# BUTSpeechFIT/VBx

Measured on NVIDIA H100. Metric: x-vectors/sec through 10 VB-HMM EM iters, higher is better.
Workload: dtype f32

## Files before the change

vbx_b200/csrc/vbx_capi.cu:

```cuda
#include <dlfcn.h>
#include <nvtx3/nvToolsExt.h>

#include <algorithm>
#include <cmath>
#include <cstdio>
#include <cstring>
#include <numeric>
#include <string>
#include <vector>

#include "../../include/vbx_b200.h"
#include "vbx_internal.cuh"

struct vbx_handle_s {
    int device = 0;
    int sms = 0;
    std::string err;
    vbx::Plan plan;
    vbx::Workspace ws;
    bool planned = false, bound = false, prepared = false;
    bool f64_only = false;
    size_t ws_need = 0;
    void *plan_mem = nullptr;
    int opt_fb_spl = 0;
    int opt_fb_classic = 0;
    int opt_projection = 0;
    int opt_timing = 0;
    int opt_gemm = 0;
    int opt_debug_sync = 0;
    int opt_fb_split = 0;
    int opt_exact_stop = 1;
    int64_t launches = 0;
    cudaStream_t hi_stream = nullptr;
    cudaEvent_t ev_fork = nullptr, ev_join = nullptr;
    int opt_graph = 0;
    cudaStream_t graph_stream = nullptr;
    cudaEvent_t ev_g0 = nullptr, ev_g1 = nullptr;
    cudaGraphExec_t graph_exec = nullptr;
    uint64_t graph_key = 0, seen_key = 0;
    int64_t graph_launches = 0;
    bool graph_broken = false;
    void *nccl_comm = nullptr;
    int nccl_ranks = 1;
    int (*nccl_allreduce)(const void *, void *, size_t, int, int, void *, cudaStream_t) = nullptr;
    std::vector<int64_t> offsets_host;
    std::vector<int64_t> ahc_d_off;
    size_t ahc_need = 0;
    std::vector<cudaEvent_t> ev_pool;
    size_t ev_used = 0;
    std::vector<int> ev_class;
    double t_ms[VBX_N_KERNEL_CLASSES] = {0};
    int64_t t_cnt[VBX_N_KERNEL_CLASSES] = {0};
};

namespace {

int fail(vbx_handle_t h, int code, const std::string &msg) {
    if (h) h->err = msg;
    return code;
}
int cuda_fail(vbx_handle_t h, cudaError_t e, const char *what) {
    return fail(h, VBX_ERR_CUDA, std::string(what) + ": " + cudaGetErrorString(e));
}
size_t align_up(size_t v, size_t a = 256) { return (v + a - 1) / a * a; }

struct Range {
    explicit Range(const char *name) { nvtxRangePushA(name); }
    ~Range() { nvtxRangePop(); }
};

struct DeviceGuard {
    int prev = -1;
    cudaError_t err = cudaSuccess;
    explicit DeviceGuard(int device) {
        if (cudaGetDevice(&prev) != cudaSuccess) prev = -1;
        if (prev != device) err = cudaSetDevice(device);
    }
    ~DeviceGuard() {
// ... 115 lines not shown
    h->device = device;
    h->sms = prop.multiProcessorCount;
    {
        DeviceGuard guard(device);
        int lo = 0, hi = 0;
        if (guard.err != cudaSuccess || cudaDeviceGetStreamPriorityRange(&lo, &hi) != cudaSuccess ||
            cudaStreamCreateWithPriority(&h->hi_stream, cudaStreamNonBlocking, hi) != cudaSuccess ||
            cudaEventCreateWithFlags(&h->ev_fork, cudaEventDisableTiming) != cudaSuccess ||
            cudaEventCreateWithFlags(&h->ev_join, cudaEventDisableTiming) != cudaSuccess ||
            cudaStreamCreateWithFlags(&h->graph_stream, cudaStreamNonBlocking) != cudaSuccess ||
            cudaEventCreateWithFlags(&h->ev_g0, cudaEventDisableTiming) != cudaSuccess ||
            cudaEventCreateWithFlags(&h->ev_g1, cudaEventDisableTiming) != cudaSuccess) {
            vbx_destroy(h);
            return VBX_ERR_CUDA;
        }
    }
    *out = h;
    return VBX_OK;
}

int vbx_destroy(vbx_handle_t h) {
    if (!h) return VBX_ERR_ARG;
    DeviceGuard guard(h->device);
    if (h->plan_mem) cudaFree(h->plan_mem);
    if (h->hi_stream) cudaStreamDestroy(h->hi_stream);
    if (h->ev_fork) cudaEventDestroy(h->ev_fork);
    if (h->ev_join) cudaEventDestroy(h->ev_join);
    if (h->graph_exec) cudaGraphExecDestroy(h->graph_exec);
    if (h->graph_stream) cudaStreamDestroy(h->graph_stream);
    if (h->ev_g0) cudaEventDestroy(h->ev_g0);
    if (h->ev_g1) cudaEventDestroy(h->ev_g1);
    for (cudaEvent_t e : h->ev_pool) cudaEventDestroy(e);
    delete h;
    return VBX_OK;
}

const char *vbx_last_error(vbx_handle_t h) { return h ? h->err.c_str() : "null handle"; }

int vbx_set_option(vbx_handle_t h, const char *name, int32_t value) {
    if (!h || !name) return VBX_ERR_ARG;
    drop_graph(h);
    if (!strcmp(name, "graph")) {
        if (value < 0 || value > 2) return fail(h, VBX_ERR_ARG, "graph must be 0 (auto), 1 (always) or 2 (never)");
        h->opt_graph = value;
        return VBX_OK;
    }
    if (!strcmp(name, "fb_states_per_lane")) {
        if (value != 0 && value != 1 && value != 2 && value != 4) return fail(h, VBX_ERR_ARG, "fb_states_per_lane must be 0,1,2,4");
        h->opt_fb_spl = value;
        return VBX_OK;
    }
    if (!strcmp(name, "fb_classic")) {
        h->opt_fb_classic = value ? 1 : 0;
        return VBX_OK;
    }
    if (!strcmp(name, "gemm")) {
        if (value != 0 && value != 1) return fail(h, VBX_ERR_ARG, "gemm must be 0 (mma 3xTF32) or 1 (FFMA)");
        h->opt_gemm = value;
        return VBX_OK;
    }
    if (!strcmp(name, "debug_sync")) {
        h->opt_debug_sync = value ? 1 : 0;
        return VBX_OK;
    }
    if (!strcmp(name, "fb_split")) {
        if (value < 0 || value > 2) return fail(h, VBX_ERR_ARG, "fb_split must be 0 (auto), 1 (always) or 2 (never)");
        h->opt_fb_split = value;
        return VBX_OK;
    }
    if (!strcmp(name, "exact_stop")) {
        h->opt_exact_stop = value ? 1 : 0;
        return VBX_OK;
    }
    if (!strcmp(name, "timing")) {
        h->opt_timing = value ? 1 : 0;
        return VBX_OK;
    }
    if (!strcmp(name, "projection")) {
        if (value < 0 || value > 2) return fail(h, VBX_ERR_ARG, "projection must be 0,1,2");
        h->opt_projection = value;
        return VBX_OK;
    }
    return fail(h, VBX_ERR_ARG, std::string("unknown option ") + name);
}

int vbx_plan(vbx_handle_t h, const int64_t *offsets_host, int32_t n_rec, int32_t R, int32_t S,
             size_t *workspace_bytes_out) {
    if (!h || !offsets_host || n_rec < 0) return fail(h, VBX_ERR_ARG, "vbx_plan: null argument");
    if (R < 4 || R > vbx::kMaxR || (R & 3)) return fail(h, VBX_ERR_ARG, "vbx_plan: R must be a multiple of 4 in [4,128]");
    if (S != 4 && S != 8 && S != 16 && S != 32 && S != 64 && S != vbx::kMaxSWide)
        return fail(h, VBX_ERR_ARG, "vbx_plan: S must come from vbx_padded_states() or vbx_padded_states_wide()");
    if (S == vbx::kMaxSWide && h->opt_fb_split == 2)
        return fail(h, VBX_ERR_ARG, "vbx_plan: S = 128 plans always take the split forward-backward schedule (there is no fused "
                                    "sweep at 128 states), so option fb_split = 2 (never) cannot be honoured");
    if (n_rec > 0 && offsets_host[0] != 0) return fail(h, VBX_ERR_ARG, "vbx_plan: offsets[0] must be 0");
    for (int b = 0; b < n_rec; ++b) {
        const int64_t T = offsets_host[b + 1] - offsets_host[b];
        if (T < 0) return fail(h, VBX_ERR_ARG, "vbx_plan: offsets must be non-decreasing");
        if (T > (int64_t)1 << 30) return fail(h, VBX_ERR_ARG, "vbx_plan: recording longer than 2^30 frames");
    }
    DeviceGuard guard(h->device);
    cudaError_t e = guard.err;
    if (e != cudaSuccess) return cuda_fail(h, e, "cudaSetDevice");

    std::vector<int32_t> order(n_rec);
    std::iota(order.begin(), order.end(), 0);
// ... 305 lines not shown
    if (warm_start && (!alpha_io || !invL_io)) return fail(h, VBX_ERR_ARG, w + ": warm_start needs alpha_io and invL_io");
    const vbx::Plan &pl = h->plan;
    if (pl.n_rec == 0) return VBX_OK;
    if (!Li_out || !n_iters_out || !flags_out || !pi_io) return fail(h, VBX_ERR_ARG, w + ": null output pointer");
    if (pl.n_frames && (!rho || !Phi || !gamma_io)) return fail(h, VBX_ERR_ARG, w + ": null pointer");
    vbx::RunParams rp;
    rp.epsilon = epsilon;
    rp.max_iters = max_iters;
    rp.hybrid = (pl.exact && epsilon > -1e300 && epsilon < 1e300 && max_iters > 1) ? 1 : 0;
    rp.warm = warm_start ? 1 : 0;

    auto enqueue = [&](cudaStream_t st) -> int {
    int rc = 0;
    {
        Timed t(h, st, VBX_K_RUN_INIT);
        rc = counted(h, vbx::launch_run_init(pl, h->ws, gamma_io, n_states, Li_out, n_iters_out, flags_out, max_iters, Fa, Fb,
                                             loop_prob, Fa_v, Fb_v, loopP_v, st), "run_init");
    }
    if (rc) return rc;
    const int rounds = max_iters + (rp.hybrid ? 1 : 0);
    const bool fb_hi = !pl.split && pl.n_rec >= 1024;
    for (int it = 0; it < rounds; ++it) {
        Range nvtx_iter("vbx_em_iteration");
        const bool given = it == 0 && warm_start;
        if (it < max_iters) {
            if (rp.hybrid) {
                Timed t(h, st, VBX_K_EXACT64);
                rc = counted(h, vbx::launch_snapshot(pl, h->ws, gamma_io, pi_io, it, st), "snapshot");
                if (rc) return rc;
            }
            if (!given) {
                Timed t(h, st, VBX_K_MSTEP);
                rc = counted(h, h->opt_gemm ? vbx::launch_mstep_partial(pl, h->ws, rho, gamma_io, st)
                                            : vbx::launch_mstep_mma(pl, h->ws, rho, gamma_io, st), "mstep_partial");
            }
            if (rc) return rc;
            {
                Timed t(h, st, VBX_K_SPEAKER_MODEL);
                rc = counted(h, vbx::launch_speaker_model(pl, h->ws, Phi, n_states, alpha_io, invL_io, given, st), "speaker_model");
            }
            if (rc) return rc;
            {
                Timed t(h, st, VBX_K_LOGLIK);
                rc = counted(h, h->opt_gemm ? vbx::launch_loglik(pl, h->ws, rho, pi_io, n_states, st) : vbx::launch_loglik_mma(pl, h->ws, rho, pi_io, n_states, st), "loglik");
            }
            if (rc) return rc;
            if (fb_hi) {
                cudaEventRecord(h->ev_fork, st);
                cudaStreamWaitEvent(h->hi_stream, h->ev_fork, 0);
            }
            {
                cudaStream_t fs = fb_hi ? h->hi_stream : st;
                Timed t(h, fs, VBX_K_FWDBWD);
                rc = counted(h, vbx::launch_forward_backward(pl, h->ws, rp, gamma_io, pi_io, n_states, Li_out, n_iters_out, flags_out, it, h->opt_fb_spl, h->opt_fb_classic, fs), "forward_backward");
            }
            if (fb_hi) {
                cudaEventRecord(h->ev_join, h->hi_stream);
                cudaStreamWaitEvent(st, h->ev_join, 0);
            }
            if (rc) return rc;
        }
        if (rp.hybrid && it > 0) {
            Timed t(h, st, VBX_K_EXACT64);
            rc = counted(h, vbx::launch_exact64_round(pl, h->ws, rp, rho, Phi, gamma_io, pi_io, n_states, alpha_io, invL_io, Li_out,
                                                      n_iters_out, flags_out, st), "exact64");
            if (rc) return rc;
        }
    }
    return VBX_OK;
    };

    cudaStream_t user = (cudaStream_t)stream;
    const bool want_graph = (h->opt_graph == 1 || (h->opt_graph == 0 && pl.split)) && !h->opt_timing && !h->opt_debug_sync &&
                            !h->graph_broken;
    if (!want_graph) return enqueue(user);
    uint64_t key = 1469598103934665603ull;
    auto mix = [&](uint64_t v) { key = (key ^ v) * 1099511628211ull; };
    auto bits = [](double d) { uint64_t u; memcpy(&u, &d, 8); return u; };
    for (const void *p : {(const void *)rho, (const void *)Phi, (const void *)gamma_io, (const void *)pi_io, (const void *)n_states,
                          (const void *)alpha_io, (const void *)invL_io, (const void *)Li_out, (const void *)n_iters_out,
                          (const void *)flags_out, (const void *)h->ws.p, (const void *)Fa_v, (const void *)Fb_v,
                          (const void *)loopP_v})
        mix((uint64_t)(uintptr_t)p);
    mix(bits(Fa)); mix(bits(Fb)); mix(bits(loop_prob)); mix(bits(epsilon)); mix((uint64_t)max_iters); mix((uint64_t)warm_start);
    if (key == 0) key = 1;
    auto replay = [&]() -> int {
        cudaEventRecord(h->ev_g0, user);
        cudaStreamWaitEvent(h->graph_stream, h->ev_g0, 0);
        const cudaError_t e = cudaGraphLaunch(h->graph_exec, h->graph_stream);
        cudaEventRecord(h->ev_g1, h->graph_stream);
        cudaStreamWaitEvent(user, h->ev_g1, 0);
        if (e != cudaSuccess) return cuda_fail(h, e, "cudaGraphLaunch");
        return VBX_OK;
    };
    if (h->graph_exec && key == h->graph_key) {
        h->launches += h->graph_launches;
        return replay();
    }
    if (key != h->seen_key) {
        h->seen_key = key;
        return enqueue(user);
    }
    drop_graph(h);
    h->seen_key = key;
    const int64_t before = h->launches;
    if (cudaStreamBeginCapture(h->graph_stream, cudaStreamCaptureModeRelaxed) != cudaSuccess) {
        cudaGetLastError();
// ... 571 lines not shown
```

vbx_b200/csrc/vbx_internal.cuh:

```cuda
#pragma once
#include <cuda_runtime.h>
#include <stdint.h>

#include <string>
#include <vector>

#define VBX_EPS_TR 1e-8f

namespace vbx {

constexpr int kLTile = 64;
constexpr int kMTile = 512;
constexpr int kLongT = 4096;
constexpr int kChunk = 256;
constexpr int kMaxR = 128;
constexpr int kMaxS = 64;
constexpr int kMaxSWide = 128;
constexpr int kTcMaxD = 2048;

struct Plan {
    int32_t n_rec = 0, R = 0, S = 0;
    int32_t exact = 0;
    int32_t split = 0;
    int64_t n_frames = 0;
// ... 88 lines not shown
    return r;
}
template <>
__device__ __forceinline__ Vec<4> ld_vec<4>(const float *p) {
    float4 t = *reinterpret_cast<const float4 *>(p);
    Vec<4> r;
    r.v[0] = t.x;
    r.v[1] = t.y;
    r.v[2] = t.z;
    r.v[3] = t.w;
    return r;
}
template <int N>
__device__ __forceinline__ Vec<N> ldg_vec(const float *p);
template <>
__device__ __forceinline__ Vec<1> ldg_vec<1>(const float *p) {
    Vec<1> r;
    r.v[0] = __ldg(p);
    return r;
}
template <>
__device__ __forceinline__ Vec<2> ldg_vec<2>(const float *p) {
    float2 t = __ldg(reinterpret_cast<const float2 *>(p));
    Vec<2> r;
    r.v[0] = t.x;
    r.v[1] = t.y;
    return r;
}
template <>
__device__ __forceinline__ Vec<4> ldg_vec<4>(const float *p) {
    float4 t = __ldg(reinterpret_cast<const float4 *>(p));
    Vec<4> r;
    r.v[0] = t.x;
    r.v[1] = t.y;
    r.v[2] = t.z;
    r.v[3] = t.w;
    return r;
}
template <int N>
__device__ __forceinline__ void st_vec(float *p, const float *v);
template <>
__device__ __forceinline__ void st_vec<1>(float *p, const float *v) {
    *p = v[0];
}
template <>
__device__ __forceinline__ void st_vec<2>(float *p, const float *v) {
    *reinterpret_cast<float2 *>(p) = make_float2(v[0], v[1]);
}
template <>
__device__ __forceinline__ void st_vec<4>(float *p, const float *v) {
    *reinterpret_cast<float4 *>(p) = make_float4(v[0], v[1], v[2], v[3]);
}

__device__ __forceinline__ int find_problem(const int64_t *__restrict__ pref, int G, int64_t x) {
    int lo = 0, hi = G;
    while (hi - lo > 1) {
        const int mid = (lo + hi) >> 1;
        if (pref[mid] <= x) lo = mid;
        else hi = mid;
    }
    return lo;
}

#endif

int launch_prepare_scale(const Plan &pl, const Workspace &ws, const float *fea, const float *Phi, float *rho,
                         cudaStream_t st);
int launch_project_ffma(const Plan &pl, const float *X, int D, const float *V, float *rho, cudaStream_t st);
int launch_g_from_rho(const Plan &pl, const Workspace &ws, const float *rho, const float *Phi, cudaStream_t st);
int launch_run_init(const Plan &pl, const Workspace &ws, const float *gamma, const int32_t *n_states, double *Li,
                    int32_t *n_iters, int32_t *flags, int max_iters, double Fa, double Fb, double loopP,
                    const double *Fa_v, const double *Fb_v, const double *loopP_v, cudaStream_t st);
int launch_mstep_partial(const Plan &pl, const Workspace &ws, const float *rho, const float *gamma, cudaStream_t st);
int launch_speaker_model(const Plan &pl, const Workspace &ws, const float *Phi,
                         const int32_t *n_states, float *alpha_io, float *invL_io, bool from_given,
                         cudaStream_t st);
int launch_loglik(const Plan &pl, const Workspace &ws, const float *rho, const float *pi, const int32_t *n_states,
                  cudaStream_t st);
int launch_forward_backward(const Plan &pl, const Workspace &ws, const RunParams &rp, float *gamma, float *pi,
                            const int32_t *n_states, double *Li, int32_t *n_iters, int32_t *flags, int iter,
                            int spl, int classic, cudaStream_t st);
int launch_elbo_trace(const Plan &pl, const double *Li, int max_iters, double *out, cudaStream_t st);
int launch_forward_backward_split(const Plan &pl, const Workspace &ws, const RunParams &rp, float *gamma, float *pi,
                                  const int32_t *n_states, int spl, cudaStream_t st);
int launch_forward_backward_long(const Plan &pl, const Workspace &ws, const RunParams &rp, float *gamma, float *pi,
                                 const int32_t *n_states, cudaStream_t st);
int launch_mstep_mma(const Plan &pl, const Workspace &ws, const float *rho, const float *gamma, cudaStream_t st);
int launch_loglik_mma(const Plan &pl, const Workspace &ws, const float *rho, const float *pi, const int32_t *n_states,
                      cudaStream_t st);
int launch_snapshot(const Plan &pl, const Workspace &ws, const float *gamma, const float *pi, int iter, cudaStream_t st);
int launch_exact64_round(const Plan &pl, const Workspace &ws, const RunParams &rp, const float *rho, const float *Phi,
                         float *gamma, float *pi, const int32_t *n_states, float *alpha_io, float *invL_io, double *Li,
                         int32_t *n_iters, int32_t *flags, cudaStream_t st);
size_t f64_workspace_bytes(const Plan &pl);
int launch_run_f64(const Plan &pl, void *workspace, const double *fea, const double *Phi, double *gamma, double *pi,
                   const int32_t *n_states, double Fa, double Fb, double loopP, int max_iters, double epsilon,
                   double *alpha_io, double *invL_io, int warm, double *Li, int32_t *n_iters, int32_t *flags,
                   cudaStream_t st);
int launch_hard_labels(const Plan &pl, const float *gamma, const int32_t *n_states, int32_t *first, int32_t *second,
                       cudaStream_t st);
int launch_hard_labels_keep(const Plan &pl, const float *gamma, const int32_t *n_states, const int32_t *keep,
                            int32_t *first, int32_t *second, double *mass, cudaStream_t st);
int launch_init_turns(const Plan &pl, const int64_t *seg, const int64_t *spk_off, const int64_t *turn_off,
                      const int64_t *turn_lo, const int64_t *turn_hi, const int64_t *turn_cum, const double *smoothing,
                      void *gamma, void *pi, bool f64, cudaStream_t st);
int launch_init_random(const Plan &pl, const uint64_t *rec_key, const uint64_t *seed, const int32_t *n_states,
                       void *gamma, void *pi, bool f64, cudaStream_t st);
int launch_fb_dense(const double *lls, const double *tr, const double *ip, int T, int S, double *post, double *tll,
                    double *lfw, double *lbw, cudaStream_t st);
int launch_score(int n_rec, const int64_t *sys_off, const int64_t *sys_lo, const int64_t *sys_hi, const int64_t *sys_join_hi,
                 const int64_t *reg_off,
                 const int64_t *reg_lo, const int64_t *reg_hi, const uint64_t *reg_mask, const uint8_t *reg_ovl,
                 const int32_t *n_ref, int n_entries, const int32_t *entry_rec, const int64_t *label_off,
                 const int32_t *labels, const int32_t *labels2,
                 const int32_t *n_labels, const int64_t *o_off, int64_t max_cells, int64_t *covered_out,
                 int64_t *fa_out, int64_t *O_out, int32_t *flags_out,
                 const int64_t *t_off, int64_t *T_out,
                 cudaStream_t st);
size_t combine_workspace_bytes(int64_t n_rec, int K, int max_labels);
int launch_combine(int64_t n_rec, const int64_t *offsets, int64_t N, const int64_t *lo, const int64_t *hi, int K,
                   const int32_t *labels, const int32_t *labels2, const int32_t *n_labels_host, int max_labels,
                   const double *weights_host, void *workspace, int32_t *labels_out, int32_t *labels2_out,
                   int32_t *order_out, double *weights_out, int64_t *D_out, int32_t *map_out, int32_t *n_global_out,
                   int32_t *flags_out, int64_t *O_out, int64_t *L_out, cudaStream_t st);
size_t ahc_workspace_bytes(const int64_t *offsets_host, int n_rec, std::vector<int64_t> *d_off_host);
int launch_ahc(const Plan &pl, const std::vector<int64_t> &d_off, const void *x, int x_is_f64, int dim, void *workspace,
               size_t workspace_bytes, double *Z_out, double *thr_out, cudaStream_t st, std::string *err);
size_t linkage_workspace_bytes(int64_t T);
void launch_linkage(const int64_t *offsets, const int64_t *d_off, int n, void *ws, double *Z_out, cudaStream_t st);
size_t link_batch_workspace_bytes(int G, const int64_t *M_host, std::vector<int64_t> *lk_off = nullptr);
int launch_link_batch(const float *fea, const float *Phi, const int32_t *spk, int64_t N, int R, const int32_t *spk_rec,
                      int G, const int64_t *M_host, const double *c_host, void *workspace, double *n_out,
                      double *F_out, double *dist_out, double *Z_out, cudaStream_t st, const double *mean,
                      const double *std);
// ... 54 lines not shown
```

vbx_b200/csrc/vbx_kernels.cu:

```cuda
#include <math_constants.h>

#include "vbx_internal.cuh"

namespace vbx {

__device__ __forceinline__ void cp_async16(void *smem, const void *gmem) {
    unsigned s = static_cast<unsigned>(__cvta_generic_to_shared(smem));
    asm volatile("cp.async.cg.shared.global [%0], [%1], 16;\n" ::"r"(s), "l"(gmem));
}
__device__ __forceinline__ void cp_async_wait_all() {
    asm volatile("cp.async.commit_group;\n" ::);
    asm volatile("cp.async.wait_group 0;\n" ::: "memory");
}

template <int LANES>
__device__ __forceinline__ float group_sum(float v) {
#pragma unroll
    for (int off = LANES / 2; off > 0; off >>= 1) v += __shfl_xor_sync(0xffffffffu, v, off);
    return v;
}
template <int LANES>
__device__ __forceinline__ float group_max(float v) {
#pragma unroll
    for (int off = LANES / 2; off > 0; off >>= 1) v = fmaxf(v, __shfl_xor_sync(0xffffffffu, v, off));
// ... 1091 lines not shown
            for (int k = 0; k < SPL; ++k) {
                b[k] = bn[k];
                kap[k] = kapn[k];
            }
            dprev = d;
            e = en;
            f = fn;
        };
        auto bchunk = [&](const int i0, Slot(&cb)[PB], Slot(&nb)[PB], const bool check) {
#pragma unroll
            for (int i = 0; i < PB; ++i) nb[i] = load_slot(i0 + PB + i + 1);
#pragma unroll
            for (int i = 0; i < PB; ++i) {
                bstep(i0 + i, cur, cb[i], check);
                cur = cb[i];
            }
#pragma unroll
            for (int k = 0; k < SPL; ++k) {
                occ[k] += (double)occf[k];
                enter[k] += (double)entf[k];
                occf[k] = 0.f;
                entf[k] = 0.f;
            }
        };
        int i0 = 0;
        for (; i0 + 2 * PB <= Tmin - 1; i0 += 2 * PB) {
            bchunk(i0, bufA, bufB, false);
            bchunk(i0 + PB, bufB, bufA, false);
        }
        for (; i0 < Tmax - 1; i0 += 2 * PB) {
            bchunk(i0, bufA, bufB, true);
            bchunk(i0 + PB, bufB, bufA, true);
        }
    }

    double pn[SPL];
    float loc = 0.f;
#pragma unroll
    for (int k = 0; k < SPL; ++k) {
        pn[k] = (double)g0[k] + (double)Q * (double)pi[k] * enter[k];
        loc += (float)pn[k];
    }
    const float tot = group_sum<LPR>(loc);
    if (live) {
#pragma unroll
        for (int k = 0; k < SPL; ++k) {
            const int s = l * SPL + k;
            pi_io[(int64_t)rec * S_PAD + s] = (float)(pn[k] / (double)tot);
            ws.occ[(int64_t)rec * S_PAD + s] = (float)occ[k];
        }
    }
}

template <int S_PAD, int SPL>
static int launch_fb_t(const Plan &pl, const Workspace &ws, const RunParams &rp, float *gamma, float *pi,
                       const int32_t *n_states, bool classic, cudaStream_t st) {
    constexpr int RPW = 32 / (S_PAD / SPL);
    const int warps = (pl.n_rec + RPW - 1) / RPW;
    const int blocks = (warps + 3) / 4;
    if (classic)
        forward_backward_kernel<S_PAD, SPL><<<blocks, 128, 0, st>>>(pl, ws, rp, gamma, pi, n_states);
    else
        forward_backward_la_kernel<S_PAD, SPL><<<blocks, 128, 0, st>>>(pl, ws, rp, gamma, pi, n_states);
    return cudaGetLastError() == cudaSuccess ? 1 : -1;
}

__global__ void __launch_bounds__(128) elbo_kernel(Plan pl, Workspace ws, RunParams rp, double *Li, int32_t *n_iters,
                                                   int32_t *flags, int iter) {
    const int rec = blockIdx.x;
    if (!ws.active[rec]) return;
    const int tid = threadIdx.x, lane = tid & 31, warp = tid >> 5;
    const int64_t f0 = pl.offsets[rec];
    const int T = (int)(pl.offsets[rec + 1] - f0);
    const float *rs = ws.rsigma + f0;
    const float *mx = ws.rowmax + f0;
    double acc = 0.0;
    for (int t = tid; t < T; t += 128) acc += (double)mx[t] - log((double)rs[t]);
    acc = warp_sum_d(acc);
    __shared__ double part[4];
    if (lane == 0) part[warp] = acc;
    __syncthreads();
    if (tid == 0) {
        double reg = 0.0;
        for (int s = 0; s < pl.S; ++s) reg += ws.regp[(int64_t)rec * pl.S + s];
        const double elbo = (part[0] + part[1]) + (part[2] + part[3]) + ws.hp[rec].dFa * ws.gsum[rec] + 0.5 * ws.hp[rec].dFb * reg;
        const double d = elbo - ws.prev_elbo[rec];
        if (rp.hybrid && iter > 0 && isfinite(elbo)) {
            const double nb = kStopNoiseC * 5.9604644775390625e-8 * fabs(elbo);
            const bool go_on = d >= rp.epsilon + kStopGuardMult * nb;
            const bool stop = d < rp.epsilon - 4.0 * nb;
            if (!go_on && !stop) {
                ws.active[rec] = 0;
                ws.active64[rec] = 1;
                if (iter == 1 && rp.warm) {
                    ws.fresh[rec] = d >= rp.epsilon + 4.0 * nb ? 1 : 2;
                } else {
                    ws.fresh[rec] = 1;
                    n_iters[rec] = iter - 1;
                }
                return;
            }
        }
        Li[(int64_t)rec * rp.max_iters + iter] = elbo;
        n_iters[rec] = iter + 1;
        int fl = flags[rec];
        if (!isfinite(elbo)) fl |= 1;
        if (iter > 0) {
            if (d < rp.epsilon) {
                ws.active[rec] = 0;
                if (iter + 1 < rp.max_iters) fl |= 4;
                if (d < 0.0) fl |= 2;
            }
        }
        ws.prev_elbo[rec] = elbo;
        flags[rec] = fl;
    }
}

__global__ void __launch_bounds__(256) elbo_trace_kernel(int n_rec, const double *__restrict__ Li, int max_iters, double *out) {
    const int it = blockIdx.x, tid = threadIdx.x;
    double s = 0.0, c = 0.0;
    for (int r = tid; r < n_rec; r += 256) {
        const double v = Li[(int64_t)r * max_iters + it];
        if (v == v) {
            s += v;
            c += 1.0;
        }
    }
    __shared__ double ss[256], cs[256];
    ss[tid] = s;
    cs[tid] = c;
    __syncthreads();
    for (int off = 128; off > 0; off >>= 1) {
        if (tid < off) {
            ss[tid] += ss[tid + off];
            cs[tid] += cs[tid + off];
        }
        __syncthreads();
    }
    if (tid == 0) {
        out[it] = ss[0];
        out[max_iters + it] = cs[0];
    }
}
int launch_elbo_trace(const Plan &pl, const double *Li, int max_iters, double *out, cudaStream_t st) {
    elbo_trace_kernel<<<max_iters, 256, 0, st>>>(pl.n_rec, Li, max_iters, out);
    return cudaGetLastError() == cudaSuccess ? 1 : -1;
}

int launch_forward_backward(const Plan &pl, const Workspace &ws, const RunParams &rp, float *gamma, float *pi,
                            const int32_t *n_states, double *Li, int32_t *n_iters, int32_t *flags, int iter,
                            int spl, int classic, cudaStream_t st) {
    if (pl.n_rec == 0) return 0;
    if (pl.split) {
        const int rs = launch_forward_backward_split(pl, ws, rp, gamma, pi, n_states, spl, st);
        if (rs < 0) return rs;
        elbo_kernel<<<pl.n_rec, 128, 0, st>>>(pl, ws, rp, Li, n_iters, flags, iter);
        return cudaGetLastError() == cudaSuccess ? rs + 1 : -1;
    }
    int rc = -1;
#define VBX_FB(S_, L_) rc = launch_fb_t<S_, L_>(pl, ws, rp, gamma, pi, n_states, classic != 0, st)
    const int S = pl.S;
    if (spl == 0) spl = (S >= 16) ? 2 : 1;
    if (S == 64 && spl < 2) spl = 2;
    if (spl > S) spl = S;
    switch (S) {
        case 4:
            if (spl == 1) VBX_FB(4, 1);
            else if (spl == 2) VBX_FB(4, 2);
            else VBX_FB(4, 4);
            break;
        case 8:
            if (spl == 1) VBX_FB(8, 1);
            else if (spl == 2) VBX_FB(8, 2);
            else VBX_FB(8, 4);
            break;
        case 16:
            if (spl == 1) VBX_FB(16, 1);
            else if (spl == 2) VBX_FB(16, 2);
            else VBX_FB(16, 4);
            break;
        case 32:
            if (spl == 1) VBX_FB(32, 1);
            else if (spl == 2) VBX_FB(32, 2);
            else VBX_FB(32, 4);
            break;
        case 64:
            if (spl == 2) VBX_FB(64, 2);
            else VBX_FB(64, 4);
            break;
        default: return -1;
    }
#undef VBX_FB
    if (rc < 0) return rc;
    const int rl = launch_forward_backward_long(pl, ws, rp, gamma, pi, n_states, st);
    if (rl < 0) return rl;
    elbo_kernel<<<pl.n_rec, 128, 0, st>>>(pl, ws, rp, Li, n_iters, flags, iter);
    return cudaGetLastError() == cudaSuccess ? rc + rl + 1 : -1;
}

}
```

vbx_b200/csrc/vbx_project_tc.cu:

```cuda
#include <cuda.h>

#include "vbx_internal.cuh"

namespace vbx {

namespace {

constexpr int kTileM = 256;
constexpr int kKB = 32;
constexpr int kVBytes = 128 * 128;
constexpr int kXBytes = kTileM * 128;
constexpr int kConsumerThreads = 256;
constexpr int kThreads = kConsumerThreads + 128;

template <int NS> struct Pipe {
    static constexpr int kStages = NS == 2 ? 3 : 2;
    static constexpr int kStageBytes = kXBytes + NS * kVBytes;
    static constexpr int kSmemBytes = 1024 + kStages * kStageBytes + 128 + 512;
};

__device__ __forceinline__ uint32_t smem_u32(const void *p) { return static_cast<uint32_t>(__cvta_generic_to_shared(p)); }

__device__ __forceinline__ void mbar_init(uint32_t bar, uint32_t count) {
    asm volatile("mbarrier.init.shared::cta.b64 [%0], %1;" ::"r"(bar), "r"(count));
}
__device__ __forceinline__ void mbar_arrive(uint32_t bar) {
    asm volatile("mbarrier.arrive.shared::cta.b64 _, [%0];" ::"r"(bar) : "memory");
}
__device__ __forceinline__ void mbar_expect_tx(uint32_t bar, uint32_t bytes) {
    asm volatile("mbarrier.arrive.expect_tx.shared::cta.b64 _, [%0], %1;" ::"r"(bar), "r"(bytes) : "memory");
}
__device__ __forceinline__ void mbar_wait(uint32_t bar, uint32_t parity) {
    asm volatile(
        "{\n\t.reg .pred p;\n\t"
        "WAIT_%=:\n\t"
        "mbarrier.try_wait.parity.shared::cta.b64 p, [%0], %1;\n\t"
        "@p bra DONE_%=;\n\t"
        "bra WAIT_%=;\n\t"
        "DONE_%=:\n\t}" ::"r"(bar),
        "r"(parity)
        : "memory");
}
__device__ __forceinline__ void bulk_g2s(uint32_t dst, const void *src, uint32_t bytes, uint32_t bar) {
    asm volatile("cp.async.bulk.shared::cluster.global.mbarrier::complete_tx::bytes [%0], [%1], %2, [%3];" ::"r"(dst),
                 "l"(src), "r"(bytes), "r"(bar)
                 : "memory");
}
__device__ __forceinline__ void tma_load_2d(uint32_t dst, const CUtensorMap *map, int c0, int c1, uint32_t bar) {
    asm volatile("cp.async.bulk.tensor.2d.shared::cluster.global.tile.mbarrier::complete_tx::bytes [%0], [%1, {%2, %3}], [%4];" ::"r"(dst),
                 "l"(reinterpret_cast<uint64_t>(map)), "r"(c0), "r"(c1), "r"(bar)
                 : "memory");
}

__device__ __forceinline__ uint64_t make_desc(uint32_t smem_addr) {
    const uint32_t lo = ((smem_addr >> 4) & 0x3fffu) | (1u << 16);
    const uint32_t hi = (1024u >> 4) | (1u << 30);
    return ((uint64_t)hi << 32) | lo;
}
__device__ __forceinline__ void wgmma_tf32(float (&d)[64], const uint32_t (&a)[4], uint64_t db, uint32_t accumulate) {
    asm volatile(
        "{\n\t.reg .pred p;\n\t"
        "setp.ne.b32 p, %69, 0;\n\t"
        "wgmma.mma_async.sync.aligned.m64n128k8.f32.tf32.tf32 "
        "{%0, %1, %2, %3, %4, %5, %6, %7, %8, %9, %10, %11, %12, %13, %14, %15, %16, %17, %18, %19, %20, %21, %22, %23, %24, %25, %26, %27, %28, %29, %30, %31, %32, %33, %34, %35, %36, %37, %38, %39, %40, %41, %42, %43, %44, %45, %46, %47, %48, %49, %50, %51, %52, %53, %54, %55, %56, %57, %58, %59, %60, %61, %62, %63}, {%64, %65, %66, %67}, %68, p, 1, 1;\n\t}"
        : "+f"(d[0]), "+f"(d[1]), "+f"(d[2]), "+f"(d[3]), "+f"(d[4]), "+f"(d[5]), "+f"(d[6]), "+f"(d[7]),
          "+f"(d[8]), "+f"(d[9]), "+f"(d[10]), "+f"(d[11]), "+f"(d[12]), "+f"(d[13]), "+f"(d[14]), "+f"(d[15]),
          "+f"(d[16]), "+f"(d[17]), "+f"(d[18]), "+f"(d[19]), "+f"(d[20]), "+f"(d[21]), "+f"(d[22]), "+f"(d[23]),
          "+f"(d[24]), "+f"(d[25]), "+f"(d[26]), "+f"(d[27]), "+f"(d[28]), "+f"(d[29]), "+f"(d[30]), "+f"(d[31]),
          "+f"(d[32]), "+f"(d[33]), "+f"(d[34]), "+f"(d[35]), "+f"(d[36]), "+f"(d[37]), "+f"(d[38]), "+f"(d[39]),
          "+f"(d[40]), "+f"(d[41]), "+f"(d[42]), "+f"(d[43]), "+f"(d[44]), "+f"(d[45]), "+f"(d[46]), "+f"(d[47]),
          "+f"(d[48]), "+f"(d[49]), "+f"(d[50]), "+f"(d[51]), "+f"(d[52]), "+f"(d[53]), "+f"(d[54]), "+f"(d[55]),
          "+f"(d[56]), "+f"(d[57]), "+f"(d[58]), "+f"(d[59]), "+f"(d[60]), "+f"(d[61]), "+f"(d[62]), "+f"(d[63])
        : "r"(a[0]), "r"(a[1]), "r"(a[2]), "r"(a[3]), "l"(db), "r"(accumulate));
}
__device__ __forceinline__ void wgmma_fence() { asm volatile("wgmma.fence.sync.aligned;" ::: "memory"); }
__device__ __forceinline__ void wgmma_commit() { asm volatile("wgmma.commit_group.sync.aligned;" ::: "memory"); }
template <int N> __device__ __forceinline__ void wgmma_wait() { asm volatile("wgmma.wait_group.sync.aligned %0;" ::"n"(N) : "memory"); }
__device__ __forceinline__ void fence_operands(float (&d)[64]) {
#pragma unroll
    for (int i = 0; i < 64; ++i) asm volatile("" : "+f"(d[i])::"memory");
}

__device__ __forceinline__ void split_rn(const float x, float &hi, float &lo) {
    const uint32_t h = (__float_as_uint(x) + 0x1000u) & 0xffffe000u;
    hi = __uint_as_float(h);
    lo = __uint_as_float((__float_as_uint(x - hi) + 0x1000u) & 0xffffe000u);
}

__device__ __forceinline__ void split3_rn(const float x, float &x1, float &x2, float &x3) {
    x1 = __uint_as_float((__float_as_uint(x) + 0x1000u) & 0xffffe000u);
    const float r1 = x - x1;
    x2 = __uint_as_float((__float_as_uint(r1) + 0x1000u) & 0xffffe000u);
    x3 = r1 - x2;
}

template <int NS>
__global__ void build_v_images_kernel(const float *__restrict__ V, int D, float *__restrict__ img) {
    const int kb = blockIdx.x;
    for (int i = threadIdx.x; i < 128 * 32; i += blockDim.x) {
        const int n = i >> 5, kk = i & 31;
// ... 347 lines not shown
```

Measured before the change: 166.1 million.

## Add TMA bulk-copy ring-buffered forward-backward kernel with checkpointed backward recompute

Adds a new forward-backward kernel in which each warp streams per-frame likelihood rows, gamma checkpoints and rsigma windows into a 3-stage shared-memory ring using cp.async.bulk and mbarriers. The backward pass recomputes forward alphas from checkpoints saved every F frames instead of reloading them. It is enabled by default for recordings up to 2048 frames with aligned gamma, replacing the lookahead kernel. The aim is to hide global-memory latency on the serial recursion, at the cost of extra shared memory, recompute work and more complex synchronisation.

New measurement: 172.3 million, median of 6. 1.04x the previous value.

```diff
diff --git a/vbx_b200/csrc/vbx_capi.cu b/vbx_b200/csrc/vbx_capi.cu
--- a/vbx_b200/csrc/vbx_capi.cu
+++ b/vbx_b200/csrc/vbx_capi.cu
@@ -24,6 +24,7 @@
     void *plan_mem = nullptr;
     int opt_fb_spl = 0;
     int opt_fb_classic = 0;
+    int opt_fb_ring = 1;
     int opt_projection = 0;
     int opt_timing = 0;
     int opt_gemm = 0;
@@ -245,6 +246,10 @@
     }
     if (!strcmp(name, "fb_classic")) {
         h->opt_fb_classic = value ? 1 : 0;
+        return VBX_OK;
+    }
+    if (!strcmp(name, "fb_ring")) {
+        h->opt_fb_ring = value ? 1 : 0;
         return VBX_OK;
     }
     if (!strcmp(name, "gemm")) {
@@ -656,7 +661,7 @@
             {
                 cudaStream_t fs = fb_hi ? h->hi_stream : st;
                 Timed t(h, fs, VBX_K_FWDBWD);
-                rc = counted(h, vbx::launch_forward_backward(pl, h->ws, rp, gamma_io, pi_io, n_states, Li_out, n_iters_out, flags_out, it, h->opt_fb_spl, h->opt_fb_classic, fs), "forward_backward");
+                rc = counted(h, vbx::launch_forward_backward(pl, h->ws, rp, gamma_io, pi_io, n_states, Li_out, n_iters_out, flags_out, it, h->opt_fb_spl, h->opt_fb_classic, h->opt_fb_ring, fs), "forward_backward");
             }
             if (fb_hi) {
                 cudaEventRecord(h->ev_join, h->hi_stream);
diff --git a/vbx_b200/csrc/vbx_internal.cuh b/vbx_b200/csrc/vbx_internal.cuh
--- a/vbx_b200/csrc/vbx_internal.cuh
+++ b/vbx_b200/csrc/vbx_internal.cuh
@@ -164,6 +164,36 @@
     *reinterpret_cast<float4 *>(p) = make_float4(v[0], v[1], v[2], v[3]);
 }
 
+__device__ __forceinline__ uint32_t smem_u32(const void *p) { return static_cast<uint32_t>(__cvta_generic_to_shared(p)); }
+__device__ __forceinline__ void mbar_init(uint32_t bar, uint32_t count) {
+    asm volatile("mbarrier.init.shared::cta.b64 [%0], %1;" ::"r"(bar), "r"(count));
+}
+__device__ __forceinline__ void mbar_arrive(uint32_t bar) {
+    asm volatile("mbarrier.arrive.shared::cta.b64 _, [%0];" ::"r"(bar) : "memory");
+}
+__device__ __forceinline__ void mbar_expect_tx(uint32_t bar, uint32_t bytes) {
+    asm volatile("mbarrier.arrive.expect_tx.shared::cta.b64 _, [%0], %1;" ::"r"(bar), "r"(bytes) : "memory");
+}
+__device__ __forceinline__ void mbar_add_tx(uint32_t bar, uint32_t bytes) {
+    asm volatile("mbarrier.expect_tx.relaxed.cta.shared::cta.b64 [%0], %1;" ::"r"(bar), "r"(bytes) : "memory");
+}
+__device__ __forceinline__ void mbar_wait(uint32_t bar, uint32_t parity) {
+    asm volatile(
+        "{\n\t.reg .pred p;\n\t"
+        "WAIT_%=:\n\t"
+        "mbarrier.try_wait.parity.shared::cta.b64 p, [%0], %1;\n\t"
+        "@p bra DONE_%=;\n\t"
+        "bra WAIT_%=;\n\t"
+        "DONE_%=:\n\t}" ::"r"(bar),
+        "r"(parity)
+        : "memory");
+}
+__device__ __forceinline__ void bulk_g2s(uint32_t dst, const void *src, uint32_t bytes, uint32_t bar) {
+    asm volatile("cp.async.bulk.shared::cluster.global.mbarrier::complete_tx::bytes [%0], [%1], %2, [%3];" ::"r"(dst),
+                 "l"(src), "r"(bytes), "r"(bar)
+                 : "memory");
+}
+
 __device__ __forceinline__ int find_problem(const int64_t *__restrict__ pref, int G, int64_t x) {
     int lo = 0, hi = G;
     while (hi - lo > 1) {
@@ -191,7 +221,7 @@
                   cudaStream_t st);
 int launch_forward_backward(const Plan &pl, const Workspace &ws, const RunParams &rp, float *gamma, float *pi,
                             const int32_t *n_states, double *Li, int32_t *n_iters, int32_t *flags, int iter,
-                            int spl, int classic, cudaStream_t st);
+                            int spl, int classic, int ring, cudaStream_t st);
 int launch_elbo_trace(const Plan &pl, const double *Li, int max_iters, double *out, cudaStream_t st);
 int launch_forward_backward_split(const Plan &pl, const Workspace &ws, const RunParams &rp, float *gamma, float *pi,
                                   const int32_t *n_states, int spl, cudaStream_t st);
diff --git a/vbx_b200/csrc/vbx_kernels.cu b/vbx_b200/csrc/vbx_kernels.cu
--- a/vbx_b200/csrc/vbx_kernels.cu
+++ b/vbx_b200/csrc/vbx_kernels.cu
@@ -1167,16 +1167,397 @@
     }
 }
 
+template <int SPL>
+struct FwdState {
+    float y[SPL];
+    float Yc, q, c, rn, rs1;
+};
+template <int SPL, int LPR>
+__device__ __forceinline__ void fwd_init(FwdState<SPL> &st, const Vec<SPL> &p0, const Vec<SPL> &p1, const float *pi,
+                                         const float *w, const int l, const bool live, const int ns, float *an) {
+    float loc = 0.f, locq = 0.f, locc = 0.f;
+#pragma unroll
+    for (int k = 0; k < SPL; ++k) {
+        const int s = l * SPL + k;
+        st.y[k] = (live && s < ns) ? p0.v[k] * (pi[k] + VBX_EPS_TR) : 0.f;
+        loc += st.y[k];
+        locq = fmaf(p1.v[k], st.y[k], locq);
+        locc = fmaf(p1.v[k], w[k], locc);
+    }
+    st.Yc = group_sum<LPR>(loc);
+    st.q = group_sum<LPR>(locq);
+    st.c = group_sum<LPR>(locc);
+    st.rn = 1.f;
+    st.rs1 = rcp_fast(st.Yc);
+#pragma unroll
+    for (int k = 0; k < SPL; ++k) an[k] = st.y[k] * st.rs1;
+}
+template <int SPL, int LPR>
+__device__ __forceinline__ float fwd_step(FwdState<SPL> &st, const Vec<SPL> &ps, const Vec<SPL> &pn, const float *w,
+                                          const float P, float *an) {
+    float ys[SPL], locq = 0.f, locc = 0.f;
+#pragma unroll
+    for (int k = 0; k < SPL; ++k) {
+        ys[k] = (st.rn * ps.v[k]) * fmaf(P, st.y[k], w[k] * st.Yc);
+        locq = fmaf(pn.v[k], ys[k], locq);
+        locc = fmaf(pn.v[k], w[k], locc);
+    }
+    const float qn = group_sum<LPR>(locq);
+    const float cn = group_sum<LPR>(locc);
+    const float Ys = st.rn * fmaf(P, st.q, st.c * st.Yc);
+    const float inv = rcp_fast(Ys);
+    const float rsig = st.rn * st.Yc * inv;
+#pragma unroll
+    for (int k = 0; k < SPL; ++k) {
+        an[k] = ys[k] * inv;
+        st.y[k] = ys[k];
+    }
+    st.Yc = Ys;
+    st.q = qn;
+    st.c = cn;
+    st.rn = st.rs1;
+    st.rs1 = rsig;
+    return rsig;
+}
+
+template <int S_PAD, int SPL>
+struct FbRing {
+    static constexpr int LPR = S_PAD / SPL, RPW = 32 / LPR;
+    static constexpr int F = (SPL == 4) ? 5 : (SPL == 2 ? 10 : 16);
+    static constexpr int FF = 2 * F;
+    static constexpr int RW = (F + 6 + 3) / 4 * 4;
+    static constexpr int GROUP = 2 * F * S_PAD + RW;
+    static constexpr int STAGE = RPW * GROUP;
+    static constexpr int kStages = 3;
+    static constexpr int kSmemBytes = 128 + 4 * kStages * STAGE * 4;
+};
+
+template <int S_PAD, int SPL>
+__global__ void __launch_bounds__(128) forward_backward_ring_kernel(Plan pl, Workspace ws, RunParams rp, float *gamma,
+                                                                    float *pi_io, const int32_t *__restrict__ n_states) {
+    using G = FbRing<S_PAD, SPL>;
+    constexpr int LPR = G::LPR, RPW = G::RPW, F = G::F, FF = G::FF, NST = G::kStages;
+    extern __shared__ __align__(128) unsigned char fb_ring_smem[];
+    const int lane = threadIdx.x & 31, warp = threadIdx.x >> 5;
+    const int warp_global = blockIdx.x * 4 + warp;
+    const int g = lane / LPR, l = lane % LPR;
+    const int slot = warp_global * RPW + g;
+    int rec = -1;
+    if (slot < pl.n_rec) rec = pl.order[slot];
+    const bool live = rec >= 0 && ws.active[rec] != 0 && pl.lrec_nchunks[rec] == 0;
+    int64_t f0 = 0;
+    int T = 0;
+    if (live) {
+        f0 = pl.offsets[rec];
+        T = (int)(pl.offsets[rec + 1] - f0);
+    }
+    int Tmax = T, Tmin = live ? T : 0x7fffffff;
+#pragma unroll
+    for (int off = 16; off > 0; off >>= 1) {
+        Tmax = max(Tmax, __shfl_xor_sync(0xffffffffu, Tmax, off));
+        Tmin = min(Tmin, __shfl_xor_sync(0xffffffffu, Tmin, off));
+    }
+    if (Tmax == 0) return;
+    const int Tlast = max(T - 1, 0);
+    const int ns = live ? (n_states ? n_states[rec] : S_PAD) : 0;
+    const float P = rec >= 0 ? ws.hp[rec].loopP : 0.f, Q = 1.f - P;
+
+    float pi[SPL], w[SPL];
+#pragma unroll
+    for (int k = 0; k < SPL; ++k) {
+        const int s = l * SPL + k;
+        const bool sl = live && s < ns;
+        pi[k] = sl ? pi_io[(int64_t)rec * S_PAD + s] : 0.f;
+        w[k] = sl ? fmaf(Q, pi[k], VBX_EPS_TR) : 0.f;
+    }
+    const float *pp = ws.p + f0 * S_PAD + l * SPL;
+    float *ga = live ? gamma + f0 * S_PAD + l * SPL : ws.scratch + l * SPL;
+    float *rs = live ? ws.rsigma + f0 : ws.scratch + kMaxS;
+    const int64_t gstr = live ? S_PAD : 0;
+    const int rstr = live ? 1 : 0;
+
+    const uint32_t bar0 = smem_u32(fb_ring_smem) + warp * NST * 8;
+    float *ring = reinterpret_cast<float *>(fb_ring_smem + 128) + warp * NST * G::STAGE;
+    if (lane == 0) {
+#pragma unroll
+        for (int i = 0; i < NST; ++i) mbar_init(bar0 + 8 * i, 1);
+        asm volatile("fence.mbarrier_init.release.cluster;" ::: "memory");
+    }
+    __syncwarp();
+    const bool issuer = live && l == 0;
+    const float *prec = ws.p + f0 * S_PAD;
+    const float *grec = gamma + f0 * S_PAD;
+    const int nf = (Tmax - 1 + FF - 1) / FF, nb = (Tmax - 1 + F - 1) / F;
+    auto stage_of = [&](const int x) { return ring + (x % NST) * G::STAGE + g * G::GROUP; };
+    auto bar_of = [&](const int x) { return bar0 + 8 * (x % NST); };
+    auto issue_fwd = [&](const int u) {
+        __syncwarp();
+        const uint32_t bar = bar_of(u);
+        if (issuer) {
+            const int lo = 2 + u * FF, n = min(FF, T - lo);
+            if (n > 0) {
+                const uint32_t bytes = (uint32_t)n * S_PAD * 4;
+                mbar_add_tx(bar, bytes);
+                bulk_g2s(smem_u32(stage_of(u)), prec + (int64_t)lo * S_PAD, bytes, bar);
+            }
+        }
+        __syncwarp();
+        if (lane == 0) mbar_arrive(bar);
+    };
+    auto rwin = [&](const int u) { return ((f0 + max(T - 1 - (u + 1) * F, 0)) & ~(int64_t)3) - f0; };
+    auto issue_bwd = [&](const int u) {
+        __syncwarp();
+        const uint32_t bar = bar_of(nf + u);
+        if (issuer) {
+            const int hi = T - 2 - u * F, lo = hi - F + 1, lc = max(lo, 0);
+            if (hi >= lc) {
+                const uint32_t rb = (uint32_t)(hi - lc + 1) * S_PAD * 4, cb = lo >= 1 ? 3 * S_PAD * 4 : 0;
+                const int64_t a0 = rwin(u), a1 = ((f0 + hi + 1 + 3) & ~(int64_t)3) - f0;
+                const uint32_t wb = (uint32_t)(a1 - a0) * 4;
+                float *dst = stage_of(nf + u);
+                mbar_add_tx(bar, rb + cb + wb);
+                bulk_g2s(smem_u32(dst + (lc - lo) * S_PAD), prec + (int64_t)lc * S_PAD, rb, bar);
+                if (cb) bulk_g2s(smem_u32(dst + F * S_PAD), grec + (int64_t)lo * S_PAD, cb, bar);
+                bulk_g2s(smem_u32(dst + 2 * F * S_PAD), ws.rsigma + f0 + a0, wb, bar);
+            }
+        }
+        __syncwarp();
+        if (lane == 0) mbar_arrive(bar);
+    };
+
+    float alast[SPL];
+    {
+        FwdState<SPL> fs;
+        {
+            const Vec<SPL> p0 = ldg_vec<SPL>(pp);
+            const Vec<SPL> p1 = ldg_vec<SPL>(pp + (int64_t)min(1, Tlast) * S_PAD);
+            for (int u = 0; u < min(NST - 1, nf); ++u) issue_fwd(u);
+            fwd_init<SPL, LPR>(fs, p0, p1, pi, w, l, live, ns, alast);
+            st_vec<SPL>(ga, alast);
+            if (l == 0) rs[0] = fs.rs1;
+        }
+        auto fstep = [&](const int j, const Vec<SPL> &ps, const Vec<SPL> &pn, const bool check) {
+            const int s = j + 1, kb = T - 1 - s;
+            if (kb >= F && kb % F == 0) {
+                sto_vec<SPL>(ga + s * gstr, fs.y);
+                if (l == 0) {
+                    const float sc[4] = {fs.Yc, fs.q, fs.c, fs.rn};
+                    sto_vec<4>(ga + (s + 1) * gstr, sc);
+                    sto_vec<1>(ga + (s + 2) * gstr, &fs.rs1);
+                }
+            }
+            float an[SPL];
+            const float rsig = fwd_step<SPL, LPR>(fs, ps, pn, w, P, an);
+            const bool act = !check || s < T;
+#pragma unroll
+            for (int k = 0; k < SPL; ++k) alast[k] = act ? an[k] : alast[k];
+            if (act) {
+                if (s == T - 1) sto_vec<SPL>(ga + s * gstr, an);
+                if (l == 0) rs[s * rstr] = rsig;
+            }
+        };
+        Vec<SPL> ps = ldg_vec<SPL>(pp + (int64_t)min(1, Tlast) * S_PAD);
+        auto fstage = [&](const int u, const float *sp, const bool check) {
+            Vec<SPL> buf[FF];
+#pragma unroll
+            for (int i = 0; i < FF; ++i) buf[i] = ld_vec<SPL>(sp + i * S_PAD);
+            if (u + NST - 1 < nf) issue_fwd(u + NST - 1);
+#pragma unroll
+            for (int i = 0; i < FF; ++i) {
+                fstep(u * FF + i, ps, buf[i], check);
+                ps = buf[i];
+            }
+        };
+        for (int u = 0; u < nf; ++u) {
+            mbar_wait(bar_of(u), (u / NST) & 1);
+            const float *sp = stage_of(u) + l * SPL;
+            if ((u + 1) * FF <= Tmin - 1)
+                fstage(u, sp, false);
+            else
+                fstage(u, sp, true);
+        }
+    }
+    asm volatile("fence.proxy.async.global;" ::: "memory");
+    __syncwarp();
+
+    for (int u = 0; u < min(NST - 1, nb); ++u) issue_bwd(u);
+    float g0[SPL], occf[SPL], entf[SPL];
+    double enter[SPL], occ[SPL];
+#pragma unroll
+    for (int k = 0; k < SPL; ++k) {
+        g0[k] = alast[k];
+        occ[k] = (double)alast[k];
+        enter[k] = 0.0;
+        occf[k] = 0.f;
+        entf[k] = 0.f;
+    }
+    {
+        float b[SPL], kap[SPL];
+        float dprev = 1.f, e = 0.f, f;
+        {
+            const Vec<SPL> pl1 = ldo_vec<SPL>(pp + (int64_t)Tlast * S_PAD);
+            const float rl1 = ldo_vec<1>(rs + Tlast * rstr).v[0];
+            float locf = 0.f;
+#pragma unroll
+            for (int k = 0; k < SPL; ++k) {
+                b[k] = 1.f;
+                kap[k] = pl1.v[k] * rl1;
+                locf = fmaf(w[k], kap[k], locf);
+            }
+            f = group_sum<LPR>(locf);
+        }
+        auto bstep = [&](const int ii, const Vec<SPL> &a, const Vec<SPL> &pt, const float rt, const bool check) {
+            const int t = T - 2 - ii;
+            float v[SPL], kapn[SPL], loce = 0.f, locf = 0.f;
+#pragma unroll
+            for (int k = 0; k < SPL; ++k) {
+                v[k] = kap[k] * b[k];
+                kapn[k] = pt.v[k] * rt;
+                const float wk = w[k] * kapn[k];
+                loce = fmaf(wk, v[k], loce);
+                locf += wk;
+            }
+            const float en = group_sum<LPR>(loce);
+            const float fn = group_sum<LPR>(locf);
+            const float d = fmaf(P, e, dprev * f);
+            float gn[SPL], bn[SPL], gs = 0.f;
+#pragma unroll
+            for (int k = 0; k < SPL; ++k) {
+                bn[k] = fmaf(P, v[k], d);
+                gn[k] = a.v[k] * bn[k];
+                gs += gn[k];
+            }
+            {
+                const float sc = rcp_fast(group_sum<LPR>(gs));
+#pragma unroll
+                for (int k = 0; k < SPL; ++k) gn[k] *= sc;
+            }
+            if (!check) {
+#pragma unroll
+                for (int k = 0; k < SPL; ++k) {
+                    g0[k] = gn[k];
+                    occf[k] += gn[k];
+                    entf[k] += v[k];
+                }
+                sto_vec<SPL>(ga + t * gstr, gn);
+            } else {
+                const bool act = t >= 0;
+#pragma unroll
+                for (int k = 0; k < SPL; ++k) {
+                    g0[k] = act ? gn[k] : g0[k];
+                    occf[k] += act ? gn[k] : 0.f;
+                    entf[k] += act ? v[k] : 0.f;
+                }
+                if (act) sto_vec<SPL>(ga + t * gstr, gn);
+            }
+#pragma unroll
+            for (int k = 0; k < SPL; ++k) {
+                b[k] = bn[k];
+                kap[k] = kapn[k];
+            }
+            dprev = d;
+            e = en;
+            f = fn;
+        };
+        auto bstage = [&](const int u, const float *st, const int rb, const bool check) {
+            const float *sp = st + l * SPL, *sr = st + 2 * F * S_PAD;
+            const int lo = T - 1 - (u + 1) * F, z = min(max(-lo, 0), F - 1);
+            Vec<SPL> pr[F];
+            float rt[F];
+#pragma unroll
+            for (int i = 0; i < F; ++i) {
+                pr[i] = ld_vec<SPL>(sp + i * S_PAD);
+                rt[i] = sr[max(rb - i, 0)];
+            }
+            FwdState<SPL> fs, f1;
+            {
+                const Vec<SPL> cy = ld_vec<SPL>(sp + F * S_PAD);
+                const Vec<4> c4 = ld_vec<4>(st + (F + 1) * S_PAD);
+                const float crs = st[(F + 2) * S_PAD];
+                const Vec<SPL> q0 = ld_vec<SPL>(sp + z * S_PAD), q1 = ld_vec<SPL>(sp + min(z + 1, F - 1) * S_PAD);
+                if (u + NST - 1 < nb) issue_bwd(u + NST - 1);
+                float a0[SPL];
+                fwd_init<SPL, LPR>(f1, q0, q1, pi, w, l, live, ns, a0);
+                const bool ck = lo >= 1;
+#pragma unroll
+                for (int k = 0; k < SPL; ++k) {
+                    fs.y[k] = ck ? cy.v[k] : f1.y[k];
+                    f1.y[k] = a0[k];
+                }
+                fs.Yc = ck ? c4.v[0] : f1.Yc;
+                fs.q = ck ? c4.v[1] : f1.q;
+                fs.c = ck ? c4.v[2] : f1.c;
+                fs.rn = ck ? c4.v[3] : f1.rn;
+                fs.rs1 = ck ? crs : f1.rs1;
+            }
+            Vec<SPL> a[F];
+#pragma unroll
+            for (int i = 0; i < F; ++i) {
+                const int s = lo + i;
+                FwdState<SPL> nx = fs;
+                fwd_step<SPL, LPR>(nx, pr[i], pr[min(i + 1, F - 1)], w, P, a[i].v);
+                if (s >= 1) fs = nx;
+#pragma unroll
+                for (int k = 0; k < SPL; ++k) a[i].v[k] = s == 0 ? f1.y[k] : a[i].v[k];
+            }
+#pragma unroll
+            for (int i = 0; i < F; ++i) bstep(u * F + i, a[F - 1 - i], pr[F - 1 - i], rt[i], check);
+#pragma unroll
+            for (int k = 0; k < SPL; ++k) {
+                occ[k] += (double)occf[k];
+                enter[k] += (double)entf[k];
+                occf[k] = 0.f;
+                entf[k] = 0.f;
+            }
+        };
+        for (int u = 0; u < nb; ++u) {
+            mbar_wait(bar_of(nf + u), ((nf + u) / NST) & 1);
+            const float *st = stage_of(nf + u);
+            const int rb = (int)min((int64_t)(T - 2 - u * F) - rwin(u), (int64_t)(G::RW - 1));
+            if ((u + 1) * F <= Tmin - 1)
+                bstage(u, st, rb, false);
+            else
+                bstage(u, st, rb, true);
+        }
+    }
+
+    double pn[SPL];
+    float loc = 0.f;
+#pragma unroll
+    for (int k = 0; k < SPL; ++k) {
+        pn[k] = (double)g0[k] + (double)Q * (double)pi[k] * enter[k];
+        loc += (float)pn[k];
+    }
+    const float tot = group_sum<LPR>(loc);
+    if (live) {
+#pragma unroll
+        for (int k = 0; k < SPL; ++k) {
+            const int s = l * SPL + k;
+            pi_io[(int64_t)rec * S_PAD + s] = (float)(pn[k] / (double)tot);
+            ws.occ[(int64_t)rec * S_PAD + s] = (float)occ[k];
+        }
+    }
+}
+
+constexpr int64_t kRingMaxT = 2048;
+
 template <int S_PAD, int SPL>
 static int launch_fb_t(const Plan &pl, const Workspace &ws, const RunParams &rp, float *gamma, float *pi,
-                       const int32_t *n_states, bool classic, cudaStream_t st) {
+                       const int32_t *n_states, bool classic, bool ring, cudaStream_t st) {
     constexpr int RPW = 32 / (S_PAD / SPL);
     const int warps = (pl.n_rec + RPW - 1) / RPW;
     const int blocks = (warps + 3) / 4;
-    if (classic)
+    if (classic) {
         forward_backward_kernel<S_PAD, SPL><<<blocks, 128, 0, st>>>(pl, ws, rp, gamma, pi, n_states);
-    else
+    } else if (ring && pl.max_T <= kRingMaxT && (reinterpret_cast<uintptr_t>(gamma) & 15) == 0) {
+        constexpr int smem = FbRing<S_PAD, SPL>::kSmemBytes;
+        if (cudaFuncSetAttribute(forward_backward_ring_kernel<S_PAD, SPL>, cudaFuncAttributeMaxDynamicSharedMemorySize,
+                                 smem) != cudaSuccess)
+            return -1;
+        forward_backward_ring_kernel<S_PAD, SPL><<<blocks, 128, smem, st>>>(pl, ws, rp, gamma, pi, n_states);
+    } else {
         forward_backward_la_kernel<S_PAD, SPL><<<blocks, 128, 0, st>>>(pl, ws, rp, gamma, pi, n_states);
+    }
     return cudaGetLastError() == cudaSuccess ? 1 : -1;
 }
 
@@ -1265,7 +1646,7 @@
 
 int launch_forward_backward(const Plan &pl, const Workspace &ws, const RunParams &rp, float *gamma, float *pi,
                             const int32_t *n_states, double *Li, int32_t *n_iters, int32_t *flags, int iter,
-                            int spl, int classic, cudaStream_t st) {
+                            int spl, int classic, int ring, cudaStream_t st) {
     if (pl.n_rec == 0) return 0;
     if (pl.split) {
         const int rs = launch_forward_backward_split(pl, ws, rp, gamma, pi, n_states, spl, st);
@@ -1274,7 +1655,7 @@
         return cudaGetLastError() == cudaSuccess ? rs + 1 : -1;
     }
     int rc = -1;
-#define VBX_FB(S_, L_) rc = launch_fb_t<S_, L_>(pl, ws, rp, gamma, pi, n_states, classic != 0, st)
+#define VBX_FB(S_, L_) rc = launch_fb_t<S_, L_>(pl, ws, rp, gamma, pi, n_states, classic != 0, ring != 0, st)
     const int S = pl.S;
     if (spl == 0) spl = (S >= 16) ? 2 : 1;
     if (S == 64 && spl < 2) spl = 2;
diff --git a/vbx_b200/csrc/vbx_project_tc.cu b/vbx_b200/csrc/vbx_project_tc.cu
--- a/vbx_b200/csrc/vbx_project_tc.cu
+++ b/vbx_b200/csrc/vbx_project_tc.cu
@@ -19,33 +19,6 @@
     static constexpr int kSmemBytes = 1024 + kStages * kStageBytes + 128 + 512;
 };
 
-__device__ __forceinline__ uint32_t smem_u32(const void *p) { return static_cast<uint32_t>(__cvta_generic_to_shared(p)); }
-
-__device__ __forceinline__ void mbar_init(uint32_t bar, uint32_t count) {
-    asm volatile("mbarrier.init.shared::cta.b64 [%0], %1;" ::"r"(bar), "r"(count));
-}
-__device__ __forceinline__ void mbar_arrive(uint32_t bar) {
-    asm volatile("mbarrier.arrive.shared::cta.b64 _, [%0];" ::"r"(bar) : "memory");
-}
-__device__ __forceinline__ void mbar_expect_tx(uint32_t bar, uint32_t bytes) {
-    asm volatile("mbarrier.arrive.expect_tx.shared::cta.b64 _, [%0], %1;" ::"r"(bar), "r"(bytes) : "memory");
-}
-__device__ __forceinline__ void mbar_wait(uint32_t bar, uint32_t parity) {
-    asm volatile(
-        "{\n\t.reg .pred p;\n\t"
-        "WAIT_%=:\n\t"
-        "mbarrier.try_wait.parity.shared::cta.b64 p, [%0], %1;\n\t"
-        "@p bra DONE_%=;\n\t"
-        "bra WAIT_%=;\n\t"
-        "DONE_%=:\n\t}" ::"r"(bar),
-        "r"(parity)
-        : "memory");
-}
-__device__ __forceinline__ void bulk_g2s(uint32_t dst, const void *src, uint32_t bytes, uint32_t bar) {
-    asm volatile("cp.async.bulk.shared::cluster.global.mbarrier::complete_tx::bytes [%0], [%1], %2, [%3];" ::"r"(dst),
-                 "l"(src), "r"(bytes), "r"(bar)
-                 : "memory");
-}
 __device__ __forceinline__ void tma_load_2d(uint32_t dst, const CUtensorMap *map, int c0, int c1, uint32_t bar) {
     asm volatile("cp.async.bulk.tensor.2d.shared::cluster.global.tile.mbarrier::complete_tx::bytes [%0], [%1, {%2, %3}], [%4];" ::"r"(dst),
                  "l"(reinterpret_cast<uint64_t>(map)), "r"(c0), "r"(c1), "r"(bar)
```
